# stella-cv/stella_vslam

Measured on NVIDIA H100. Metric: frames/sec (ORB+match+local BA) @1920x1080, 2000 kpts, higher is better.
Workload: dtype u8

## Files before the change

### stella_vslam_b200/csrc/lba_kernels.cu

```cuda
#include <algorithm>
#include <cmath>
#include <cstdlib>
#include <new>
#include <sched.h>

#include <chrono>
#include <memory>
#include <mutex>
#include <thread>
#include <vector>

#include "common.cuh"
#include "lm_common.cuh"
#include "quat.cuh"
#include "staging.cuh"
#include "track_chain.cuh"

namespace b200 {
namespace lba {

constexpr double kPi = 3.14159265358979323846;

struct Cam {
    int model;
// ... 773 lines not shown
                int x = 0, rem = tid;
                while (rem >= 6 - x) {
                    rem -= 6 - x;
                    ++x;
                }
                const int y = x + rem;
                W.Hpp[(size_t)i * 36 + x * 6 + y] = r;
                W.Hpp[(size_t)i * 36 + y * 6 + x] = r;
            } else {
                W.bp[(size_t)i * 6 + (tid - 21)] = r;
            }
        }
    }
    if (!last_cta_arrives(W.tickets, n_rows, &last_flag)) return;
    lm_after_build(W, stage);
}

__device__ __forceinline__ void dmma_m8n8k4(double& c0, double& c1, double a, double b) {
    asm volatile("mma.sync.aligned.m8n8k4.row.col.f64.f64.f64.f64 {%0,%1}, {%2}, {%3}, {%0,%1};" : "+d"(c0), "+d"(c1) : "d"(a), "d"(b));
}

__device__ __forceinline__ void schur_finish_block(const WinDev& W, const SchurBlock sb, double lambda, int lane) {
    const double* __restrict__ partials = W.chunk_part;
    double* __restrict__ M = W.M;
    const int n = W.n, ld = W.ld;
    for (int el = lane; el < 42; el += 32) {
        if (el >= 36 && sb.i != sb.j) continue;
        double sacc = 0.0;
        for (int c = sb.chunk_start; c < sb.chunk_end; ++c) sacc += __ldcg(partials + (size_t)c * 42 + el);
        if (el < 36) {
            const int r = el / 6, c = el - r * 6;
            double val = -sacc;
            if (sb.i == sb.j) val += W.Hpp[(size_t)sb.i * 36 + el] + (r == c ? lambda : 0.0);
            M[(size_t)(6 * sb.j + c) * ld + 6 * sb.i + r] = val;
            if (sb.i == sb.j) M[(size_t)(6 * sb.i + r) * ld + 6 * sb.j + c] = val;
        } else {
            const int r = el - 36;
            M[(size_t)n * ld + 6 * sb.i + r] = W.bp[(size_t)sb.i * 6 + r] - sacc;
        }
    }
}

__device__ void se3_oplus(const double* q, const double* t, const double* upd, double* qo, double* to) {
    const double* om = upd;
    const double* up = upd + 3;
    const double theta = sqrt(om[0] * om[0] + om[1] * om[1] + om[2] * om[2]);
    const double O[9] = {0, -om[2], om[1], om[2], 0, -om[0], -om[1], om[0], 0};
    double O2[9];
    for (int i = 0; i < 3; ++i)
        for (int j = 0; j < 3; ++j) O2[i * 3 + j] = O[i * 3] * O[j] + O[i * 3 + 1] * O[3 + j] + O[i * 3 + 2] * O[6 + j];
    double a, b, c, d;
    if (theta < 0.00001) {
        a = 1.0; b = 0.5; c = 0.5; d = 1.0 / 6.0;
    } else {
        a = sin(theta) / theta;
        b = (1 - cos(theta)) / (theta * theta);
        c = b;
        d = (theta - sin(theta)) / (theta * theta * theta);
    }
    double R[9], V[9];
    for (int i = 0; i < 9; ++i) {
        const double I = (i % 4 == 0) ? 1.0 : 0.0;
        R[i] = I + a * O[i] + b * O2[i];
        V[i] = I + c * O[i] + d * O2[i];
    }
    double dq[4], dt[3];
    rot_to_quat(R, dq);
    quat_normalize(dq);
    for (int i = 0; i < 3; ++i) dt[i] = V[i * 3] * up[0] + V[i * 3 + 1] * up[1] + V[i * 3 + 2] * up[2];
    double uv[3] = {dq[1] * t[2] - dq[2] * t[1], dq[2] * t[0] - dq[0] * t[2], dq[0] * t[1] - dq[1] * t[0]};
    uv[0] += uv[0]; uv[1] += uv[1]; uv[2] += uv[2];
    to[0] = dt[0] + t[0] + dq[3] * uv[0] + (dq[1] * uv[2] - dq[2] * uv[1]);
    to[1] = dt[1] + t[1] + dq[3] * uv[1] + (dq[2] * uv[0] - dq[0] * uv[2]);
    to[2] = dt[2] + t[2] + dq[3] * uv[2] + (dq[0] * uv[1] - dq[1] * uv[0]);
    double nq[4];
    nq[3] = dq[3] * q[3] - dq[0] * q[0] - dq[1] * q[1] - dq[2] * q[2];
    nq[0] = dq[3] * q[0] + dq[0] * q[3] + dq[1] * q[2] - dq[2] * q[1];
    nq[1] = dq[3] * q[1] + dq[1] * q[3] + dq[2] * q[0] - dq[0] * q[2];
    nq[2] = dq[3] * q[2] + dq[2] * q[3] + dq[0] * q[1] - dq[1] * q[0];
    quat_normalize(nq);
    qo[0] = nq[0]; qo[1] = nq[1]; qo[2] = nq[2]; qo[3] = nq[3];
}

constexpr int kCholThreads = 512;
constexpr int kNB = 24;
constexpr int kCholCluster = 8;

__device__ __forceinline__ unsigned cluster_ctarank() {
    unsigned r;
    asm volatile("mov.u32 %0, %%cluster_ctarank;" : "=r"(r));
    return r;
}
__device__ __forceinline__ unsigned cluster_nctarank() {
    unsigned r;
    asm volatile("mov.u32 %0, %%cluster_nctarank;" : "=r"(r));
    return r;
}
__device__ __forceinline__ void cluster_sync_all() {
    asm volatile("barrier.cluster.arrive.release.aligned;\n\tbarrier.cluster.wait.acquire.aligned;" ::: "memory");
}

__global__ void __launch_bounds__(kCholThreads) chol_solve_kernel(const WinDev* __restrict__ wins) {
    const unsigned crank = cluster_ctarank(), csize = cluster_nctarank();
    const WinDev& W = wins[blockIdx.x / csize];
    const LmCtl* __restrict__ ctl = W.ctl;
    if (!ctl->outer_go) return;
    const int n = W.n, ld = W.ld, K = W.K;
    double* __restrict__ M = W.M;
    const double* __restrict__ bp = W.bp;
    double* __restrict__ xp = W.xp;
    const int* __restrict__ pose_col = W.pose_col;
    double* __restrict__ result = W.r_result;
    int* __restrict__ fail = W.fail;
    extern __shared__ __align__(32) double dyn[];
    const double lambda = ctl->lambda;
    const int cur_idx = ctl->cur & 1;
    const double* __restrict__ q_cur = W.q[cur_idx];
    const double* __restrict__ t_cur = W.t[cur_idx];
    double* __restrict__ q_new = W.q[cur_idx ^ 1];
    double* __restrict__ t_new = W.t[cur_idx ^ 1];
    double* __restrict__ Rt_new = W.Rt[cur_idx ^ 1];
    double* D = dyn;
    double* Pn = dyn + kNB * (kNB + 1);
    const int mp = (n + 1 + 3) & ~3;
    __shared__ double xs[1024];
    __shared__ double invd_all[1024];
    __shared__ double sh[kCholThreads];
    __shared__ int bad;
    const int tid = threadIdx.x, nt = blockDim.x;
    const bool lead = crank == 0;
    if (tid == 0) bad = *fail;
    __syncthreads();
    long long t_diag = 0, t_panel = 0, t_trail = 0, t_back = 0, t0 = clock64(), t1;
#define PHASE(acc) do { t1 = clock64(); acc += t1 - t0; t0 = t1; } while (0)
    for (int kb = 0; kb < n && !bad; kb += kNB) {
        const int nb = min(kNB, n - kb);
        if (tid < 32) {
            double r[kNB];
#pragma unroll
            for (int k = 0; k < kNB; ++k) r[k] = (tid < nb && k <= tid) ? M[(size_t)(kb + tid) * ld + kb + k] : ((k == tid) ? 1.0 : 0.0);
            int b = 0;
#pragma unroll
            for (int j = 0; j < kNB; ++j) {
                const double djj = __shfl_sync(0xFFFFFFFFu, r[j], j);
                b |= (!(djj > 0.0) || !isfinite(djj)) ? 1 : 0;
                const double inv = rsqrt(djj), dd = djj * inv;
                if (tid == 0) invd_all[kb + j] = inv;
                r[j] = (tid == j) ? dd : ((tid > j) ? r[j] * inv : r[j]);
                const double mine = (tid > j) ? r[j] : 0.0;
#pragma unroll
                for (int k = j + 1; k < kNB; ++k) {
                    const double lkj = __shfl_sync(0xFFFFFFFFu, r[j], k);
                    r[k] = fma(-((tid >= k) ? mine : 0.0), lkj, r[k]);
                }
            }
            if (tid < kNB) {
#pragma unroll
                for (int k = 0; k < kNB; ++k) {
                    D[tid * (kNB + 1) + k] = r[k];
                }
            }
            if (tid == 0 && b) bad = 1;
        }
        __syncthreads();
        PHASE(t_diag);
        if (bad) break;
        const int r0 = kb + nb, m = n + 1 - r0;
        for (int t = tid; t < m; t += nt) {
            double* row = M + (size_t)(r0 + t) * ld + kb;
            double x[kNB];
#pragma unroll
            for (int j = 0; j < kNB; ++j) x[j] = (j < nb) ? row[j] : 0.0;
#pragma unroll
            for (int j = 0; j < kNB; ++j) {
                x[j] *= invd_all[kb + j];
#pragma unroll
                for (int k = j + 1; k < kNB; ++k) x[k] = fma(-x[j], D[k * (kNB + 1) + j], x[k]);
            }
#pragma unroll
            for (int j = 0; j < kNB; ++j) {
                Pn[(size_t)j * mp + t] = x[j];
            }
        }
        for (int idx = tid; idx < kNB * 4; idx += nt) {
            const int j = idx >> 2, t = m + (idx & 3);
            if (t < mp) Pn[(size_t)j * mp + t] = 0.0;
        }
        __syncthreads();
        PHASE(t_panel);
        const int tm = (m + 3) >> 2;
        const int n_tiles = tm * (tm + 1) / 2;
        for (int tile = tid * csize + crank; tile < n_tiles; tile += nt * csize) {
            int tr = (int)((sqrt(8.0 * tile + 1.0) - 1.0) * 0.5);
            while ((tr + 1) * (tr + 2) / 2 <= tile) ++tr;
            while (tr * (tr + 1) / 2 > tile) --tr;
            const int tc = tile - tr * (tr + 1) / 2;
            double acc[16];
#pragma unroll
            for (int a = 0; a < 16; ++a) acc[a] = 0.0;
            const int rb = tr * 4, cb = tc * 4;
#pragma unroll 4
            for (int k = 0; k < kNB; ++k) {
                const double2* pa = reinterpret_cast<const double2*>(Pn + (size_t)k * mp + rb);
                const double2* pb = reinterpret_cast<const double2*>(Pn + (size_t)k * mp + cb);
                const double2 a0 = pa[0], a1 = pa[1], b0 = pb[0], b1 = pb[1];
                const double a[4] = {a0.x, a0.y, a1.x, a1.y}, b[4] = {b0.x, b0.y, b1.x, b1.y};
#pragma unroll
                for (int u = 0; u < 4; ++u)
#pragma unroll
                    for (int w = 0; w < 4; ++w) acc[u * 4 + w] = fma(a[u], b[w], acc[u * 4 + w]);
            }
#pragma unroll
            for (int u = 0; u < 4; ++u)
#pragma unroll
                for (int w = 0; w < 4; ++w) {
                    const int r = rb + u, c = cb + w;
                    if (r < m && c <= r && r0 + c < n) M[(size_t)(r0 + r) * ld + r0 + c] -= acc[u * 4 + w];
                }
        }
        __syncthreads();
        if (csize > 1) cluster_sync_all();
        if (lead) {
            for (int idx = tid; idx < nb * nb; idx += nt) {
                const int i = idx / nb, j = idx - i * nb;
                if (j <= i) M[(size_t)(kb + i) * ld + kb + j] = D[i * (kNB + 1) + j];
            }
            for (int idx = tid; idx < m * nb; idx += nt) {
                const int t = idx / nb, j = idx - t * nb;
                M[(size_t)(r0 + t) * ld + kb + j] = Pn[(size_t)j * mp + t];
            }
        }
        __syncthreads();
        PHASE(t_trail);
    }
    if (!lead) return;
    if (bad) {
        if (tid == 0) {
            *fail = 1;
            result[0] = 0.0;
        }
    } else {
        for (int i = tid; i < n; i += nt) xs[i] = M[(size_t)n * ld + i];
        __syncthreads();
        for (int kb = ((n - 1) / kNB) * kNB; kb >= 0; kb -= kNB) {
            const int nb = min(kNB, n - kb);
            for (int idx = tid; idx < kNB * kNB; idx += nt) {
                const int i = idx / kNB, j = idx - i * kNB;
                D[i * (kNB + 1) + j] = (i < nb && j <= i) ? M[(size_t)(kb + i) * ld + kb + j] : 0.0;
            }
            __syncthreads();
            if (tid < 32) {
                double y = (tid < nb) ? xs[kb + tid] : 0.0;
#pragma unroll
                for (int j = kNB - 1; j >= 0; --j) {
                    const double xj = __shfl_sync(0xFFFFFFFFu, y, j) * ((j < nb) ? invd_all[kb + j] : 0.0);
                    if (tid == j) y = xj;
                    else if (tid < j) y = fma(-D[j * (kNB + 1) + tid], xj, y);
                }
                if (tid < nb) xs[kb + tid] = y;
            }
            __syncthreads();
            for (int i = tid; i < kb; i += nt) {
                double sacc = xs[i];
                for (int k = 0; k < nb; ++k) sacc = fma(-M[(size_t)(kb + k) * ld + i], xs[kb + k], sacc);
                xs[i] = sacc;
            }
            __syncthreads();
        }
        double sc = 0.0;
        for (int i = tid; i < n; i += nt) {
            xp[i] = xs[i];
            sc += xs[i] * (lambda * xs[i] + bp[i]);
        }
        const double tot = block_sum(sc, sh);
        PHASE(t_back);
        if (tid == 0) {
            result[0] = 1.0;
            result[1] = tot;
            result[2] = (double)t_diag;
            result[3] = (double)t_panel;
            result[4] = (double)t_trail;
            result[5] = (double)t_back;
        }
    }
#undef PHASE
    __syncthreads();
    for (int k = tid; k < K; k += nt) {
        double qn[4], tn[3];
        const int pc = pose_col[k];
        if (pc >= 0 && !bad) {
            se3_oplus(q_cur + 4 * k, t_cur + 3 * k, xs + 6 * pc, qn, tn);
        } else {
            for (int i = 0; i < 4; ++i) qn[i] = q_cur[4 * k + i];
            for (int i = 0; i < 3; ++i) tn[i] = t_cur[3 * k + i];
        }
        for (int i = 0; i < 4; ++i) q_new[4 * k + i] = qn[i];
        for (int i = 0; i < 3; ++i) t_new[3 * k + i] = tn[i];
        double R[9];
        quat_to_rot(qn, R);
        for (int i = 0; i < 9; ++i) Rt_new[12 * k + i] = R[i];
        for (int i = 0; i < 3; ++i) Rt_new[12 * k + 9 + i] = tn[i];
    }
}

constexpr int kSmmaKS = 100;
constexpr int kSmmaWarpDoubles = (6 + 7) * kSmmaKS;
__global__ void __launch_bounds__(128) schur_mma_kernel(const WinDev* __restrict__ wins) {
    extern __shared__ __align__(16) double smma[];
    const WinDev& W = wins[blockIdx.y];
    const LmCtl* ctl = W.ctl;
    if (!ctl->outer_go) return;
    const int warp = threadIdx.x >> 5, lane = threadIdx.x & 31;
    const int wid = blockIdx.x * 4 + warp;
    const int n_blocks = W.n_blocks, n_chunks = W.blk_chunk_start[n_blocks];
    if (wid >= n_chunks) {
        const int e = wid - n_chunks;
        if (e < n_blocks) {
            const SchurBlock sb = W.blocks[e];
            if (sb.chunk_start == sb.chunk_end) schur_finish_block(W, sb, ctl->lambda, lane);
        }
        return;
    }
    double* As = smma + (size_t)warp * kSmmaWarpDoubles;
    double* Bs = As + 6 * kSmmaKS;
    const SchurChunk ch = W.chunks[wid];
    const int Lf = W.Lf;
    const double* __restrict__ Hpl = W.Hpl;
    const double* __restrict__ Dinv = W.Dinv;
    const int g = lane >> 2, t4 = lane & 3;
    const double* a_row = As + min(g, 5) * kSmmaKS + t4;
    const double* b_row = Bs + min(g, 6) * kSmmaKS + t4;
    double c0 = 0.0, c1 = 0.0;
    for (int base = ch.start; base < ch.end; base += 32) {
        const int k = base + lane;
        const int np = min(32, ch.end - base);
        {
            double t[18], hc[18], b3[3];
            if (k < ch.end) {
                const int4 pr = W.pairs[k];
                double ra[12], rc[12], ha[18];
                load_hpl_record(Hpl + (size_t)pr.x * kHplStride, ra);
                load_hpl_record(Hpl + (size_t)pr.y * kHplStride, rc);
                expand_hpl(ra, ha);
                expand_hpl(rc, hc);
                const int lc = pr.z;
                const double D0 = Dinv[lc], D1 = Dinv[(size_t)Lf + lc], D2 = Dinv[(size_t)2 * Lf + lc];
                const double D4 = Dinv[(size_t)3 * Lf + lc], D5 = Dinv[(size_t)4 * Lf + lc], D8 = Dinv[(size_t)5 * Lf + lc];
#pragma unroll
                for (int r = 0; r < 6; ++r) {
                    t[r * 3] = ha[r * 3] * D0 + ha[r * 3 + 1] * D1 + ha[r * 3 + 2] * D2;
                    t[r * 3 + 1] = ha[r * 3] * D1 + ha[r * 3 + 1] * D4 + ha[r * 3 + 2] * D5;
                    t[r * 3 + 2] = ha[r * 3] * D2 + ha[r * 3 + 1] * D5 + ha[r * 3 + 2] * D8;
                }
                b3[0] = b3[1] = b3[2] = 0.0;
                if (ch.diag) {
                    b3[0] = W.bl[lc];
                    b3[1] = W.bl[(size_t)Lf + lc];
                    b3[2] = W.bl[(size_t)2 * Lf + lc];
                }
            } else {
#pragma unroll
                for (int i = 0; i < 18; ++i) t[i] = hc[i] = 0.0;
                b3[0] = b3[1] = b3[2] = 0.0;
            }
            double* ap = As + 3 * lane;
            double* bp2 = Bs + 3 * lane;
#pragma unroll
            for (int r = 0; r < 6; ++r)
#pragma unroll
                for (int kk = 0; kk < 3; ++kk) {
                    ap[r * kSmmaKS + kk] = t[r * 3 + kk];
                    bp2[r * kSmmaKS + kk] = hc[r * 3 + kk];
                }
#pragma unroll
            for (int kk = 0; kk < 3; ++kk) bp2[6 * kSmmaKS + kk] = b3[kk];
        }
        __syncwarp();
        const int steps = (3 * np + 3) >> 2;
#pragma unroll 4
        for (int s2 = 0; s2 < steps; ++s2) dmma_m8n8k4(c0, c1, a_row[4 * s2], b_row[4 * s2]);
        __syncwarp();
    }
    double* part = W.chunk_part + (size_t)wid * 42;
    if (g < 6) {
        if (t4 < 3) {
// ... 838 lines not shown
        }
        if (K) std::memcpy(hs + o.pose_col, h.pose_col.data(), sizeof(int) * K);
        if (L) {
            std::memcpy(hs + o.pt_col, h.pt_col.data(), sizeof(int) * L);
            std::memcpy(hs + o.pts0, P.points, sizeof(double) * 3 * L);
        }
        double* q0 = reinterpret_cast<double*>(hs + o.q0);
        double* t0 = reinterpret_cast<double*>(hs + o.t0);
        double* Rt0 = reinterpret_cast<double*>(hs + o.Rt0);
        for (size_t k = 0; k < K; ++k) {
            const double* M = P.pose_cw + 16 * k;
            const double R[9] = {M[0], M[1], M[2], M[4], M[5], M[6], M[8], M[9], M[10]};
            rot_to_quat(R, &q0[4 * k]);
            quat_normalize(&q0[4 * k]);
            t0[3 * k] = M[3]; t0[3 * k + 1] = M[7]; t0[3 * k + 2] = M[11];
            quat_to_rot(&q0[4 * k], &Rt0[12 * k]);
            Rt0[12 * k + 9] = M[3]; Rt0[12 * k + 10] = M[7]; Rt0[12 * k + 11] = M[11];
        }
        WinDev& W = hwd[x];
        std::memset(&W, 0, sizeof(W));
        W.K = h.K; W.L = h.L; W.E = h.E; W.Kf = h.Kf; W.Lf = h.Lf; W.n = h.n; W.ld = h.ld; W.n_cams = P.n_cams; W.lbc = h.lbc;
        W.e_pose = (const int*)(d + o.e_pose); W.e_point = (const int*)(d + o.e_point); W.e_cam = d + o.e_cam; W.e_robust = d + o.e_robust;
        W.e_can_outlier = d + o.e_can; W.e_obs = (const float*)(d + o.e_obs); W.e_isig = (const float*)(d + o.e_isig);
        W.e_delta = (const float*)(d + o.e_delta); W.pose_col = (const int*)(d + o.pose_col); W.pt_col = (const int*)(d + o.pt_col);
        W.cams = (const Cam*)(d + o.cams);
        W.pt_cnt = (int*)(d + o.pt_cnt); W.pt_start = (int*)(d + o.pt_start); W.order = (int*)(d + o.order); W.edges = (EdgeS*)(d + o.edges);
        W.epcol = (int*)(d + o.epcol); W.pose_cnt = (int*)(d + o.pose_cnt); W.pose_start = (int*)(d + o.pose_start);
        W.pose_edges = (int*)(d + o.pose_edges); W.level = d + o.level; W.robust = d + o.robust;
        W.rowrec = (int4*)(d + o.rowrec);
        W.lm_mask = (unsigned long long*)(d + o.lm_mask); W.mask_words = h.mask_words; W.n_blocks = h.n_blocks; W.blk_cnt = (int*)(d + o.blk_cnt);
        W.blk_pair_start = (int*)(d + o.blk_pair_start); W.blk_chunk_start = (int*)(d + o.blk_chunk_start); W.pairs = (int4*)(d + o.pairs);
        W.blocks = (SchurBlock*)(d + o.blocks); W.chunks = (SchurChunk*)(d + o.chunks); W.chunk_part = (double*)(d + o.chunk_part);
        W.blk_done = (int*)(d + o.blk_done);
        W.q[0] = (double*)(d + o.q0); W.q[1] = (double*)(d + o.q1); W.t[0] = (double*)(d + o.t0); W.t[1] = (double*)(d + o.t1);
        W.Rt[0] = (double*)(d + o.Rt0); W.Rt[1] = (double*)(d + o.Rt1); W.pts[0] = (double*)(d + o.pts0); W.pts[1] = (double*)(d + o.pts1);
        W.chi[0] = (double*)(d + o.chi0); W.chi[1] = (double*)(d + o.chi1);
        W.Hpl = (double*)(d + o.Hpl); W.Hll = (double*)(d + o.Hll); W.bl = (double*)(d + o.bl); W.Dinv = (double*)(d + o.Dinv);
        W.Hpp = (double*)(d + o.Hpp); W.bp = (double*)(d + o.bp); W.M = (double*)(d + o.M); W.xp = (double*)(d + o.xp);
        W.gP = (double*)(d + o.gP); W.gD = (double*)(d + o.gD); W.ginvd = (double*)(d + o.ginvd);
        W.r_chi = (double*)(d + o.r_chi); W.r_diag = (double*)(d + o.r_diag); W.r_scale = (double*)(d + o.r_scale); W.r_result = (double*)(d + o.r_result);
        W.fail = (int*)(d + o.fail); W.tickets = (int*)(d + o.tickets); W.bad_input = (int*)(d + o.bad);
        W.ctl = (LmCtl*)(d + o_ctl) + x;
        W.qf = (double*)(d + o.qf); W.tf = (double*)(d + o.tf); W.pf = (double*)(d + o.pf); W.out = d + o.out;
        LmCtl& c = hctl0[x];
        std::memset(&c, 0, sizeof(c));
        c.ok = 1;
        S.h_abort[x] = 0;
        c.abort_word = (stops && stops[act[x]]) ? S.d_abort + x : nullptr;
    }
    if (debug) fprintf(stderr, "[lba] %d windows staged in %.3f ms (upload %.2f MB, arena %.1f MB)\n", nw, ms_since(t_begin), upload_bytes / 1e6, cv.end / 1e6);
    cudaStream_t st = S.stream;
    int launches = 0;
    S.prof_kind.clear();
    auto mark = [&](int kind) -> int {
        if (!S.profile) return B200_OK;
        const size_t idx = S.prof_kind.size();
        if (idx >= S.prof_ev.size()) {
            cudaEvent_t e;
            B200_CUDA(cudaEventCreate(&e));
            S.prof_ev.push_back(e);
        }
        B200_CUDA(cudaEventRecord(S.prof_ev[idx], st));
        S.prof_kind.push_back(kind);
        return B200_OK;
    };
    B200_CUDA(cudaEventRecord(S.ev0, st));
    B200_CUDA(S.arena.upload(upload_bytes, st));
    B200_CUDA(cudaMemsetAsync(d + upload_bytes, 0, zero_end - upload_bytes, st));
    if ((rc = mark(-1))) return rc;
    const WinDev* wins = (const WinDev*)(d + o_wins);
    const LmCtl* d_ctl = (const LmCtl*)(d + o_ctl);
    plan_count_kernel<<<dim3(ceil_div(maxE, 256), nw), 256, 0, st>>>(wins);
    plan_scan_kernel<<<nw, 1024, 0, st>>>(wins);
    plan_place_kernel<<<dim3(ceil_div(maxE, 256), nw), 256, 0, st>>>(wins);
    plan_sort_kernel<<<dim3(ceil_div(maxL, 128), nw), 128, 0, st>>>(wins);
    plan_pose_lists_kernel<<<dim3(maxKf, nw), kListThreads, 0, st>>>(wins);
    plan_pairs_kernel<false><<<dim3(ceil_div(max_blocks, 4), nw), 128, 0, st>>>(wins);
    plan_pair_scan_kernel<<<nw, 1024, 0, st>>>(wins);
    plan_pairs_kernel<true><<<dim3(ceil_div(max_blocks, 4), nw), 128, 0, st>>>(wins);
    launches += 8;
    if ((rc = mark(0))) return rc;
    B200_RANGE("b200:lba:rounds+export");
    const bool large = max_n > kCholOnChipMax || S.force_offchip;
    const size_t chol_smem = sizeof(double) * ((size_t)kNB * (kNB + 1) + 4 + (size_t)((std::min(max_n, kCholOnChipMax) + 1 + 3) & ~3) * kNB);
    B200_CUDA(cudaFuncSetAttribute(chol_solve_kernel, cudaFuncAttributeMaxDynamicSharedMemorySize, (int)chol_smem));
    const int chol_cluster = S.chol_cluster_pinned ? S.chol_cluster : (nw <= 2 ? 8 : 4);
    auto launch_rep = [&]() -> int {
        int rcm;
        landmark_kernel<kBuild><<<dim3(max_lbc, nw), kLmThreads, 0, st>>>(wins);
        if ((rcm = mark(1))) return rcm;
        pose_rows_kernel<<<dim3(maxKf, nw), kRowThreads, 0, st>>>(wins);
        if ((rcm = mark(2))) return rcm;
        schur_mma_kernel<<<dim3(ceil_div(max_chunk_warps, 4), nw), 128, 4 * kSmmaWarpDoubles * sizeof(double), st>>>(wins);
        if ((rcm = mark(3))) return rcm;
        if (large) {
            for (int kb = 0; kb < max_n; kb += kNB) {
                const int m = max_n + 1 - std::min(kb + kNB, max_n);
                const long long tm = (m + 3) >> 2, n_tiles = tm * (tm + 1) / 2;
                gchol_panel_kernel<<<dim3(ceil_div(m + 4, kGcholThreads), nw), kGcholThreads, 0, st>>>(wins, kb);
                gchol_trail_kernel<<<dim3((unsigned)std::max<long long>(1, (n_tiles + kGcholThreads - 1) / kGcholThreads), nw), kGcholThreads, 0, st>>>(wins, kb);
                launches += 2;
            }
            gchol_finish_kernel<<<nw, kGfinThreads, 0, st>>>(wins);
        } else {
            cudaLaunchConfig_t cfg = {};
            cfg.gridDim = dim3(chol_cluster * nw);
            cfg.blockDim = dim3(kCholThreads);
            cfg.dynamicSmemBytes = chol_smem;
            cfg.stream = st;
            cudaLaunchAttribute attr[1];
            attr[0].id = cudaLaunchAttributeClusterDimension;
            attr[0].val.clusterDim.x = chol_cluster;
            attr[0].val.clusterDim.y = 1;
            attr[0].val.clusterDim.z = 1;
            cfg.attrs = attr;
            cfg.numAttrs = 1;
            B200_CUDA(cudaLaunchKernelEx(&cfg, chol_solve_kernel, wins));
        }
        if ((rcm = mark(4))) return rcm;
        backsub_kernel<<<dim3(max_lbc, nw), 128, 0, st>>>(wins);
        if ((rcm = mark(5))) return rcm;
        launches += 5;
        return B200_OK;
    };
    auto fetch_issue = [&](int b) -> int {
        B200_CUDA(cudaMemcpyAsync(h_ctl2[b], d_ctl, sizeof(LmCtl) * nw, cudaMemcpyDeviceToHost, st));
        B200_CUDA(cudaEventRecord(S.ev_ctl[b], st));
        return B200_OK;
    };
    auto fetch_wait = [&](int b) -> int {
        B200_CUDA(S.wait_event(S.ev_ctl[b]));
        h_ctl = h_ctl2[b];
        for (int x = 0; x < nw; ++x)
            if (stops && stops[act[x]] && *stops[act[x]]) S.h_abort[x] = 1;
        return B200_OK;
    };
    auto fetch_ctl = [&]() -> int {
        int r_ = fetch_issue(0);
        return r_ ? r_ : fetch_wait(0);
    };
    const int iters[2] = {iters1, iters2};
    int rc2;
    for (int r = 0; r < rounds; ++r) {
        if (r == 1) {
            if ((rc2 = fetch_ctl())) return rc2;
            for (int x = 0; x < nw; ++x) {
                volatile uint8_t* f = stops ? stops[act[x]] : nullptr;
                if (!f) continue;
                if (h_ctl[x].stop_flag || *f) {
                    S.h_abort[x] = 1;
                    *f = 1;
                } else {
                    S.h_abort[x] = 0;
                }
            }
        }
        lm_round_begin_kernel<<<ceil_div(nw, 64), 64, 0, st>>>(wins, nw, iters[r], r, gain_thr);
        ++launches;
        if (r == 1) {
            outlier_kernel<<<dim3(ceil_div(maxE, 128), nw), 128, 0, st>>>(wins, 0);
            ++launches;
        }
        if (iters[r] > 0) {
            int need = iters[r];
            for (;;) {
                const int chunk = std::max(1, std::min(need, 6));
                for (int i = 0; i < chunk; ++i)
                    if ((rc2 = launch_rep())) return rc2;
                if ((rc2 = fetch_ctl())) return rc2;
                need = 0;
                for (int x = 0; x < nw; ++x)
                    if (h_ctl[x].outer_go) need = std::max(need, std::max(1, h_ctl[x].iterations - h_ctl[x].it));
                if (need == 0) break;
            }
        }
        landmark_kernel<kRoundEnd><<<dim3(max_lbc, nw), kLmThreads, 0, st>>>(wins);
        lm_round_end_kernel<<<nw, 256, 0, st>>>(wins, r);
        launches += 2;
    }
    if (rounds == 2) outlier_kernel<<<dim3(ceil_div(maxE, 128), nw), 128, 0, st>>>(wins, 1);
    lm_export_kernel<<<dim3(ceil_div(std::max(std::max(4 * maxK, 3 * maxL), 1), 256), nw), 256, 0, st>>>(wins);
    launches += 2;
    B200_CUDA(cudaGetLastError());
    if ((rc = mark(7))) return rc;
    B200_CUDA(cudaEventRecord(S.ev1, st));
    B200_CUDA(cudaMemcpyAsync(h_export, d + export_begin, export_bytes, cudaMemcpyDeviceToHost, st));
    std::vector<int> h_bad(nw, 0);
    if ((rc2 = fetch_ctl())) return rc2;
    for (int x = 0; x < nw; ++x) B200_CUDA(cudaMemcpyAsync(&h_bad[x], d + wo[x].bad, sizeof(int), cudaMemcpyDeviceToHost, st));
    B200_CUDA(cudaStreamSynchronize(st));
    B200_CUDA(cudaEventElapsedTime(&S.last_ms, S.ev0, S.ev1));
    S.last_launches = launches;
    for (int k2 = 0; k2 < 8; ++k2) {
        S.prof_ms[k2] = 0.f;
        S.prof_n[k2] = 0;
    }
    for (size_t m = 1; m < S.prof_kind.size(); ++m) {
        float ms = 0.f;
        B200_CUDA(cudaEventElapsedTime(&ms, S.prof_ev[m - 1], S.prof_ev[m]));
        const int kd = S.prof_kind[m];
        if (kd >= 0 && kd < 8) {
            S.prof_ms[kd] += ms;
            S.prof_n[kd] += 1;
        }
    }
    if (debug) fprintf(stderr, "[lba] batch of %d windows: %.3f ms wall, %.3f ms on the stream, %d launches\n", nw, ms_since(t_begin), S.last_ms, launches);
    for (int x = 0; x < nw; ++x) {
        const int w = act[x];
        const HostWin& h = hw[x];
        const b200_lba_problem_t& P = Ps[w];
        const WinOff& o = wo[x];
        if (h_bad[x]) {
            set_error("b200_lba_solve: edge %d of window %d references an invalid vertex/camera", h_bad[x] - 1, w);
            status[w] = B200_ERR_INVALID;
            ret = B200_ERR_INVALID;
            continue;
        }
        const LmCtl& c = h_ctl[x];
        if (stats) {
            stats[w].lambda_init = c.lambda_init;
            for (int r = 0; r < 2; ++r) {
                stats[w].iterations[r] = c.iters_done[r];
                stats[w].chi2[r] = c.chi2[r];
                stats[w].lambda_final[r] = c.lambda_final[r];
            }
        }
        if (stops && stops[w] && c.stop_flag) *stops[w] = 1;
        S.last_gain_stop = c.stop_flag != 0;
        const unsigned char* ex = h_export + (o.qf - export_begin);
        const double* qf = reinterpret_cast<const double*>(ex);
        const double* tf = reinterpret_cast<const double*>(h_export + (o.tf - export_begin));
        const double* pf = reinterpret_cast<const double*>(h_export + (o.pf - export_begin));
        const unsigned char* out = h_export + (o.out - export_begin);
        int n_out = 0;
        for (int e = 0; e < h.E && rounds == 2; ++e) n_out += out[e];
        if (rounds == 2 && outlier_outs && outlier_outs[w] && h.E) std::memcpy(outlier_outs[w], out, h.E);
        if (stats) stats[w].n_outliers = n_out;
        if (h.L) std::memcpy(points_outs[w], pf, sizeof(double) * 3 * (size_t)h.L);
        for (int k = 0; k < h.K; ++k) {
            double* M = pose_outs[w] + 16 * (size_t)k;
            if (P.pose_fixed[k]) {
                std::memcpy(M, P.pose_cw + 16 * (size_t)k, sizeof(double) * 16);
                continue;
            }
            double R[9];
            quat_to_rot(&qf[4 * k], R);
            M[0] = R[0]; M[1] = R[1]; M[2] = R[2]; M[3] = tf[3 * k];
            M[4] = R[3]; M[5] = R[4]; M[6] = R[5]; M[7] = tf[3 * k + 1];
            M[8] = R[6]; M[9] = R[7]; M[10] = R[8]; M[11] = tf[3 * k + 2];
            M[12] = 0; M[13] = 0; M[14] = 0; M[15] = 1;
        }
    }
    return ret;
}

constexpr int kTrackEdgeThreads = 256;
constexpr int kMatchedBias = 1 << 30;
__global__ void __launch_bounds__(kTrackEdgeThreads) track_edges_kernel(chain::TrackShared sh, const chain::TrackFrameDev* __restrict__ frames,
                                                                        PoseProb* __restrict__ probs, PoseEdge* __restrict__ edges_all,
                                                                        int* __restrict__ edge_kp_all) {
    __shared__ int warp_sum[kTrackEdgeThreads / 32];
    __shared__ int s_base;
    const chain::TrackFrameDev& F = frames[blockIdx.x];
    const int tid = threadIdx.x, lane = tid & 31, warp = tid >> 5;
    const int n = F.status[0];
    int* slot = F.kp_landmark_out;
    for (int i = tid; i < F.kp_cap; i += kTrackEdgeThreads) {
        int l = -1;
        if (i < n && F.kp_landmark && i < F.n_kp_in) {
            l = F.kp_landmark[i];
            if (l < 0 || l >= F.n_lm) l = -1;
        }
        slot[i] = l;
        F.kp_outlier[i] = 0;
    }
    __syncthreads();
    for (int q = tid; q < F.n_lm; q += kTrackEdgeThreads) {
        const int k = F.match_out[q];
        if (k >= 0 && k < n) atomicMax(&slot[k], q + kMatchedBias);
    }
    __syncthreads();
    if (tid == 0) s_base = 0;
    const PoseProb pb = probs[blockIdx.x];
    PoseEdge* __restrict__ edges = edges_all + pb.edge_off;
    int* __restrict__ edge_kp = edge_kp_all + pb.edge_off;
    __syncthreads();
    for (int i0 = 0; i0 < n; i0 += kTrackEdgeThreads) {
        const int i = i0 + tid;
        int l = -1;
// ... 345 lines not shown
```

Baseline: 10130.

## Add shared-memory-resident two-CTA cluster Cholesky for small reduced systems

Adds a Cholesky kernel for reduced camera systems up to a size threshold. The lower triangle is held as 8x8 tiles in distributed shared memory, split by tile row across a two-CTA cluster. Panel rows are mirrored into the peer CTA's buffer, and the trailing update uses DMMA m8n8k4 tensor-core ops with split arrive/wait so local work overlaps the cluster barrier. This is meant to remove repeated global-memory traffic on the Schur matrix during factorization, at the cost of more shared memory, cluster barriers and more complex indexing. Pose-update code is factored into a helper, and a debug printout of cycle counts is added.

```diff
diff --git a/stella_vslam_b200/csrc/lba_kernels.cu b/stella_vslam_b200/csrc/lba_kernels.cu
--- a/stella_vslam_b200/csrc/lba_kernels.cu
+++ b/stella_vslam_b200/csrc/lba_kernels.cu
@@ -879,6 +879,31 @@
     qo[0] = nq[0]; qo[1] = nq[1]; qo[2] = nq[2]; qo[3] = nq[3];
 }
 
+__device__ void trial_states(const WinDev& W, const double* xs, bool solved) {
+    const int cur_idx = W.ctl->cur & 1;
+    const double* __restrict__ q_cur = W.q[cur_idx];
+    const double* __restrict__ t_cur = W.t[cur_idx];
+    double* __restrict__ q_new = W.q[cur_idx ^ 1];
+    double* __restrict__ t_new = W.t[cur_idx ^ 1];
+    double* __restrict__ Rt_new = W.Rt[cur_idx ^ 1];
+    for (int k = threadIdx.x; k < W.K; k += blockDim.x) {
+        double qn[4], tn[3];
+        const int pc = W.pose_col[k];
+        if (pc >= 0 && solved) {
+            se3_oplus(q_cur + 4 * k, t_cur + 3 * k, xs + 6 * pc, qn, tn);
+        } else {
+            for (int i = 0; i < 4; ++i) qn[i] = q_cur[4 * k + i];
+            for (int i = 0; i < 3; ++i) tn[i] = t_cur[3 * k + i];
+        }
+        for (int i = 0; i < 4; ++i) q_new[4 * k + i] = qn[i];
+        for (int i = 0; i < 3; ++i) t_new[3 * k + i] = tn[i];
+        double R[9];
+        quat_to_rot(qn, R);
+        for (int i = 0; i < 9; ++i) Rt_new[12 * k + i] = R[i];
+        for (int i = 0; i < 3; ++i) Rt_new[12 * k + 9 + i] = tn[i];
+    }
+}
+
 constexpr int kCholThreads = 512;
 constexpr int kNB = 24;
 constexpr int kCholCluster = 8;
@@ -895,6 +920,38 @@
 }
 __device__ __forceinline__ void cluster_sync_all() {
     asm volatile("barrier.cluster.arrive.release.aligned;\n\tbarrier.cluster.wait.acquire.aligned;" ::: "memory");
+}
+__device__ __forceinline__ void cluster_arrive() { asm volatile("barrier.cluster.arrive.release.aligned;" ::: "memory"); }
+__device__ __forceinline__ void cluster_wait() { asm volatile("barrier.cluster.wait.acquire.aligned;" ::: "memory"); }
+__device__ __forceinline__ double* cluster_map(double* p, unsigned rank) {
+    unsigned long long q;
+    asm volatile("mapa.u64 %0, %1, %2;" : "=l"(q) : "l"(p), "r"(rank));
+    return reinterpret_cast<double*>(q);
+}
+
+__device__ __forceinline__ bool diag_block_factor(double (&r)[kNB], int lane, double* invd, double* D) {
+    int b = 0;
+#pragma unroll
+    for (int j = 0; j < kNB; ++j) {
+        const double djj = __shfl_sync(0xFFFFFFFFu, r[j], j);
+        b |= (!(djj > 0.0) || !isfinite(djj)) ? 1 : 0;
+        const double inv = rsqrt(djj), dd = djj * inv;
+        if (lane == 0) invd[j] = inv;
+        r[j] = (lane == j) ? dd : ((lane > j) ? r[j] * inv : r[j]);
+        const double mine = (lane > j) ? r[j] : 0.0;
+#pragma unroll
+        for (int k = j + 1; k < kNB; ++k) {
+            const double lkj = __shfl_sync(0xFFFFFFFFu, r[j], k);
+            r[k] = fma(-((lane >= k) ? mine : 0.0), lkj, r[k]);
+        }
+    }
+    if (lane < kNB) {
+#pragma unroll
+        for (int k = 0; k < kNB; ++k) {
+            D[lane * (kNB + 1) + k] = r[k];
+        }
+    }
+    return b != 0;
 }
 
 __global__ void __launch_bounds__(kCholThreads) chol_solve_kernel(const WinDev* __restrict__ wins) {
@@ -902,21 +959,14 @@
     const WinDev& W = wins[blockIdx.x / csize];
     const LmCtl* __restrict__ ctl = W.ctl;
     if (!ctl->outer_go) return;
-    const int n = W.n, ld = W.ld, K = W.K;
+    const int n = W.n, ld = W.ld;
     double* __restrict__ M = W.M;
     const double* __restrict__ bp = W.bp;
     double* __restrict__ xp = W.xp;
-    const int* __restrict__ pose_col = W.pose_col;
     double* __restrict__ result = W.r_result;
     int* __restrict__ fail = W.fail;
     extern __shared__ __align__(32) double dyn[];
     const double lambda = ctl->lambda;
-    const int cur_idx = ctl->cur & 1;
-    const double* __restrict__ q_cur = W.q[cur_idx];
-    const double* __restrict__ t_cur = W.t[cur_idx];
-    double* __restrict__ q_new = W.q[cur_idx ^ 1];
-    double* __restrict__ t_new = W.t[cur_idx ^ 1];
-    double* __restrict__ Rt_new = W.Rt[cur_idx ^ 1];
     double* D = dyn;
     double* Pn = dyn + kNB * (kNB + 1);
     const int mp = (n + 1 + 3) & ~3;
@@ -936,28 +986,7 @@
             double r[kNB];
 #pragma unroll
             for (int k = 0; k < kNB; ++k) r[k] = (tid < nb && k <= tid) ? M[(size_t)(kb + tid) * ld + kb + k] : ((k == tid) ? 1.0 : 0.0);
-            int b = 0;
-#pragma unroll
-            for (int j = 0; j < kNB; ++j) {
-                const double djj = __shfl_sync(0xFFFFFFFFu, r[j], j);
-                b |= (!(djj > 0.0) || !isfinite(djj)) ? 1 : 0;
-                const double inv = rsqrt(djj), dd = djj * inv;
-                if (tid == 0) invd_all[kb + j] = inv;
-                r[j] = (tid == j) ? dd : ((tid > j) ? r[j] * inv : r[j]);
-                const double mine = (tid > j) ? r[j] : 0.0;
-#pragma unroll
-                for (int k = j + 1; k < kNB; ++k) {
-                    const double lkj = __shfl_sync(0xFFFFFFFFu, r[j], k);
-                    r[k] = fma(-((tid >= k) ? mine : 0.0), lkj, r[k]);
-                }
-            }
-            if (tid < kNB) {
-#pragma unroll
-                for (int k = 0; k < kNB; ++k) {
-                    D[tid * (kNB + 1) + k] = r[k];
-                }
-            }
-            if (tid == 0 && b) bad = 1;
+            if (diag_block_factor(r, tid, invd_all + kb, D) && tid == 0) bad = 1;
         }
         __syncthreads();
         PHASE(t_diag);
@@ -1082,22 +1111,224 @@
     }
 #undef PHASE
     __syncthreads();
-    for (int k = tid; k < K; k += nt) {
-        double qn[4], tn[3];
-        const int pc = pose_col[k];
-        if (pc >= 0 && !bad) {
-            se3_oplus(q_cur + 4 * k, t_cur + 3 * k, xs + 6 * pc, qn, tn);
-        } else {
-            for (int i = 0; i < 4; ++i) qn[i] = q_cur[4 * k + i];
-            for (int i = 0; i < 3; ++i) tn[i] = t_cur[3 * k + i];
-        }
-        for (int i = 0; i < 4; ++i) q_new[4 * k + i] = qn[i];
-        for (int i = 0; i < 3; ++i) t_new[3 * k + i] = tn[i];
-        double R[9];
-        quat_to_rot(qn, R);
-        for (int i = 0; i < 9; ++i) Rt_new[12 * k + i] = R[i];
-        for (int i = 0; i < 3; ++i) Rt_new[12 * k + 9 + i] = tn[i];
-    }
+    trial_states(W, xs, !bad);
+}
+
+constexpr int kResCluster = 2;
+constexpr int kCholResidentMax = 288;
+constexpr int kResRows = kCholResidentMax + kNB;
+
+__host__ __device__ __forceinline__ int res_tile_off(int i, int rank) {
+    const int k = (i - rank) >> 1;
+    return k * k + k * rank;
+}
+__host__ __device__ __forceinline__ int res_tix(int r, int c) { return r * 8 + (c ^ ((r & 2) << 1)); }
+__device__ __forceinline__ int tri_row(int t, int b) {
+    int a = (int)((sqrtf((float)(b * b + 4 * t)) - (float)b) * 0.5f);
+    while ((a + 1) * (a + 1) + (a + 1) * b <= t) ++a;
+    while (a > 0 && a * a + a * b > t) --a;
+    return a;
+}
+
+static size_t chol_resident_smem(int n) {
+    const int T0 = (n + 7) / 8;
+    int own = 0;
+    for (int rank = 0; rank < kResCluster; ++rank) {
+        int c = 0;
+        for (int i = rank; i <= T0; i += kResCluster) c += i < T0 ? i + 1 : T0;
+        own = std::max(own, c);
+    }
+    return sizeof(double) * 64 * ((size_t)3 * (T0 / 2 + 1) + own);
+}
+
+__global__ void __launch_bounds__(kCholThreads) chol_resident_kernel(const WinDev* __restrict__ wins) {
+    const int crank = (int)cluster_ctarank();
+    const WinDev& W = wins[blockIdx.x / kResCluster];
+    const LmCtl* __restrict__ ctl = W.ctl;
+    if (!ctl->outer_go) return;
+    const int n = W.n, ld = W.ld;
+    const double* __restrict__ M = W.M;
+    const double* __restrict__ bp = W.bp;
+    double* __restrict__ xp = W.xp;
+    double* __restrict__ result = W.r_result;
+    int* __restrict__ fail = W.fail;
+    const double lambda = ctl->lambda;
+    extern __shared__ __align__(32) double dyn[];
+    __shared__ double D[kNB * (kNB + 1)];
+    __shared__ double invd_all[kResRows];
+    __shared__ double xs[kResRows];
+    __shared__ double sh[kCholThreads];
+    __shared__ int bad;
+    const int T0 = (n + 7) >> 3;
+    double* xbuf = dyn;
+    double* tiles = dyn + (size_t)3 * 64 * (T0 / 2 + 1);
+    double* peer_xbuf = cluster_map(xbuf, crank ^ 1);
+    double* peer_tiles = cluster_map(tiles, crank ^ 1);
+    auto tile_of = [&](int i, int c) -> double* {
+        return ((i & 1) == crank ? tiles : peer_tiles) + (size_t)(res_tile_off(i, i & 1) + c) * 64;
+    };
+    const int tid = threadIdx.x, nt = blockDim.x, warp = tid >> 5, lane = tid & 31, nwarps = nt >> 5;
+    const int g = lane >> 2, t4 = lane & 3;
+    const bool lead = crank == 0;
+    if (tid == 0) bad = *fail;
+    long long t_diag = 0, t_panel = 0, t_trail = 0, t_back = 0, t0 = clock64(), t1;
+#define PHASE(acc) do { t1 = clock64(); acc += t1 - t0; t0 = t1; } while (0)
+    const int last_row = T0 - ((T0 - crank) & 1);
+    const int n_own = last_row < crank ? 0 : res_tile_off(last_row, crank) + (last_row < T0 ? last_row + 1 : T0);
+    for (int tb = warp; tb < n_own; tb += 4 * nwarps) {
+        double v[8];
+#pragma unroll
+        for (int u = 0; u < 4; ++u) {
+            const int t = tb + u * nwarps;
+            const int k = tri_row(t, crank), i = crank + 2 * k, c = t - res_tile_off(i, crank);
+#pragma unroll
+            for (int h = 0; h < 2; ++h) {
+                const int r = (lane >> 3) + 4 * h, R = 8 * i + r, C = 8 * c + (lane & 7);
+                double x = 0.0;
+                if (t < n_own) {
+                    if (i == T0) x = (r == 0 && C < n) ? M[(size_t)n * ld + C] : 0.0;
+                    else x = (R < n && C <= R) ? M[(size_t)R * ld + C] : (R == C ? 1.0 : 0.0);
+                }
+                v[2 * u + h] = x;
+            }
+        }
+#pragma unroll
+        for (int u = 0; u < 4; ++u) {
+            const int t = tb + u * nwarps;
+            if (t < n_own)
+#pragma unroll
+                for (int h = 0; h < 2; ++h) tiles[(size_t)t * 64 + res_tix((lane >> 3) + 4 * h, lane & 7)] = v[2 * u + h];
+        }
+    }
+    cluster_sync_all();
+    PHASE(t_panel);
+    for (int c0 = 0; c0 < T0 && !bad; c0 += 3) {
+        const int nbt = min(3, T0 - c0), kb = 8 * c0, nb = 8 * nbt, i1 = c0 + nbt;
+        if (tid < 32) {
+            double r[kNB];
+            const double* row = tid < nb ? tile_of(c0 + (tid >> 3), c0) : nullptr;
+#pragma unroll
+            for (int k = 0; k < kNB; ++k) r[k] = (tid < nb && k <= tid) ? row[(k >> 3) * 64 + res_tix(tid & 7, k & 7)] : ((k == tid) ? 1.0 : 0.0);
+            if (diag_block_factor(r, tid, invd_all + kb, D) && tid == 0) bad = 1;
+        }
+        __syncthreads();
+        PHASE(t_diag);
+        if (bad) break;
+        const int i0 = i1 + ((i1 ^ crank) & 1);
+        const int n_rows = i0 <= T0 ? (T0 - i0) / 2 + 1 : 0;
+        for (int t = tid; t < 8 * n_rows; t += nt) {
+            const int i = i0 + 2 * (t >> 3), rr = t & 7;
+            double* tp = tiles + (size_t)(res_tile_off(i, crank) + c0) * 64;
+            double* pp = peer_xbuf + (size_t)(i >> 1) * 3 * 64;
+            double x[kNB];
+#pragma unroll
+            for (int j = 0; j < kNB; ++j) x[j] = (j < nb) ? tp[(j >> 3) * 64 + res_tix(rr, j & 7)] : 0.0;
+#pragma unroll
+            for (int j = 0; j < kNB; ++j) {
+                x[j] *= invd_all[kb + j];
+#pragma unroll
+                for (int k = j + 1; k < kNB; ++k) x[k] = fma(-x[j], D[k * (kNB + 1) + j], x[k]);
+            }
+#pragma unroll
+            for (int j = 0; j < kNB; ++j) {
+                if (j < nb) {
+                    const int e = (j >> 3) * 64 + res_tix(rr, j & 7);
+                    tp[e] = x[j];
+                    pp[e] = x[j];
+                }
+            }
+        }
+        __syncthreads();
+        cluster_arrive();
+        PHASE(t_panel);
+        const int lb = i0 - i1;
+        const int n_trail = n_rows == 0 ? 0 : (n_rows - 1) * (n_rows - 1) + (n_rows - 1) * lb + (min(i0 + 2 * (n_rows - 1), T0 - 1) - i1 + 1);
+        for (int pass = 0; pass < 2; ++pass) {
+            if (pass == 1) cluster_wait();
+            for (int t = warp; t < n_trail; t += nwarps) {
+                const int a = tri_row(t, lb), i = i0 + 2 * a, j = i1 + t - (a * a + a * lb);
+                const bool own_j = ((j ^ crank) & 1) == 0;
+                if (own_j != (pass == 0)) continue;
+                const double* at = tiles + (size_t)(res_tile_off(i, crank) + c0) * 64;
+                const double* bt = own_j ? tiles + (size_t)(res_tile_off(j, crank) + c0) * 64 : xbuf + (size_t)(j >> 1) * 3 * 64;
+                double s0 = 0.0, s1 = 0.0;
+#pragma unroll
+                for (int s = 0; s < 6; ++s) {
+                    if (s < 2 * nbt) {
+                        const int e = (s >> 1) * 64 + res_tix(g, 4 * (s & 1) + t4);
+                        dmma_m8n8k4(s0, s1, at[e], bt[e]);
+                    }
+                }
+                double2* cp = reinterpret_cast<double2*>(tiles + (size_t)(res_tile_off(i, crank) + j) * 64 + res_tix(g, 2 * t4));
+                double2 cv = *cp;
+                cv.x -= s0;
+                cv.y -= s1;
+                *cp = cv;
+            }
+        }
+        for (int idx = tid; idx < nb * nb; idx += nt) {
+            const int i = idx / nb, j = idx - i * nb, ti = c0 + (i >> 3);
+            if (j <= i && (ti & 1) == crank) tiles[(size_t)(res_tile_off(ti, crank) + c0 + (j >> 3)) * 64 + res_tix(i & 7, j & 7)] = D[i * (kNB + 1) + j];
+        }
+        cluster_sync_all();
+        PHASE(t_trail);
+    }
+    if (lead && !bad) {
+        for (int i = tid; i < n; i += nt) xs[i] = tile_of(T0, i >> 3)[res_tix(0, i & 7)];
+        __syncthreads();
+        for (int kb = ((n - 1) / kNB) * kNB; kb >= 0; kb -= kNB) {
+            const int nb = min(kNB, n - kb), c0 = kb >> 3;
+            for (int idx = tid; idx < kNB * kNB; idx += nt) {
+                const int i = idx / kNB, j = idx - i * kNB;
+                D[i * (kNB + 1) + j] = (i < nb && j <= i) ? tile_of(c0 + (i >> 3), c0 + (j >> 3))[res_tix(i & 7, j & 7)] : 0.0;
+            }
+            __syncthreads();
+            if (tid < 32) {
+                double y = (tid < nb) ? xs[kb + tid] : 0.0;
+#pragma unroll
+                for (int j = kNB - 1; j >= 0; --j) {
+                    const double xj = __shfl_sync(0xFFFFFFFFu, y, j) * ((j < nb) ? invd_all[kb + j] : 0.0);
+                    if (tid == j) y = xj;
+                    else if (tid < j) y = fma(-D[j * (kNB + 1) + tid], xj, y);
+                }
+                if (tid < nb) xs[kb + tid] = y;
+            }
+            __syncthreads();
+            for (int i = tid; i < kb; i += nt) {
+                double sacc = xs[i];
+                for (int k = 0; k < nb; ++k) sacc = fma(-tile_of(c0 + (k >> 3), i >> 3)[res_tix(k & 7, i & 7)], xs[kb + k], sacc);
+                xs[i] = sacc;
+            }
+            __syncthreads();
+        }
+    }
+    cluster_sync_all();
+    if (!lead) return;
+    if (bad) {
+        if (tid == 0) {
+            *fail = 1;
+            result[0] = 0.0;
+        }
+    } else {
+        double sc = 0.0;
+        for (int i = tid; i < n; i += nt) {
+            xp[i] = xs[i];
+            sc += xs[i] * (lambda * xs[i] + bp[i]);
+        }
+        const double tot = block_sum(sc, sh);
+        PHASE(t_back);
+        if (tid == 0) {
+            result[0] = 1.0;
+            result[1] = tot;
+            result[2] = (double)t_diag;
+            result[3] = (double)t_panel;
+            result[4] = (double)t_trail;
+            result[5] = (double)t_back;
+        }
+    }
+#undef PHASE
+    __syncthreads();
+    trial_states(W, xs, !bad);
 }
 
 constexpr int kSmmaKS = 100;
@@ -2102,8 +2333,11 @@
     if ((rc = mark(0))) return rc;
     B200_RANGE("b200:lba:rounds+export");
     const bool large = max_n > kCholOnChipMax || S.force_offchip;
+    const bool resident = !large && max_n <= kCholResidentMax;
     const size_t chol_smem = sizeof(double) * ((size_t)kNB * (kNB + 1) + 4 + (size_t)((std::min(max_n, kCholOnChipMax) + 1 + 3) & ~3) * kNB);
+    const size_t res_smem = chol_resident_smem(std::min(max_n, kCholResidentMax));
     B200_CUDA(cudaFuncSetAttribute(chol_solve_kernel, cudaFuncAttributeMaxDynamicSharedMemorySize, (int)chol_smem));
+    B200_CUDA(cudaFuncSetAttribute(chol_resident_kernel, cudaFuncAttributeMaxDynamicSharedMemorySize, (int)res_smem));
     const int chol_cluster = S.chol_cluster_pinned ? S.chol_cluster : (nw <= 2 ? 8 : 4);
     auto launch_rep = [&]() -> int {
         int rcm;
@@ -2123,19 +2357,21 @@
             }
             gchol_finish_kernel<<<nw, kGfinThreads, 0, st>>>(wins);
         } else {
+            const int csize = resident ? kResCluster : chol_cluster;
             cudaLaunchConfig_t cfg = {};
-            cfg.gridDim = dim3(chol_cluster * nw);
+            cfg.gridDim = dim3(csize * nw);
             cfg.blockDim = dim3(kCholThreads);
-            cfg.dynamicSmemBytes = chol_smem;
+            cfg.dynamicSmemBytes = resident ? res_smem : chol_smem;
             cfg.stream = st;
             cudaLaunchAttribute attr[1];
             attr[0].id = cudaLaunchAttributeClusterDimension;
-            attr[0].val.clusterDim.x = chol_cluster;
+            attr[0].val.clusterDim.x = csize;
             attr[0].val.clusterDim.y = 1;
             attr[0].val.clusterDim.z = 1;
             cfg.attrs = attr;
             cfg.numAttrs = 1;
-            B200_CUDA(cudaLaunchKernelEx(&cfg, chol_solve_kernel, wins));
+            if (resident) B200_CUDA(cudaLaunchKernelEx(&cfg, chol_resident_kernel, wins));
+            else B200_CUDA(cudaLaunchKernelEx(&cfg, chol_solve_kernel, wins));
         }
         if ((rcm = mark(4))) return rcm;
         backsub_kernel<<<dim3(max_lbc, nw), 128, 0, st>>>(wins);
@@ -2225,6 +2461,11 @@
         }
     }
     if (debug) fprintf(stderr, "[lba] batch of %d windows: %.3f ms wall, %.3f ms on the stream, %d launches\n", nw, ms_since(t_begin), S.last_ms, launches);
+    for (int x = 0; debug && !large && x < nw; ++x) {
+        double rr[8];
+        B200_CUDA(cudaMemcpy(rr, d + wo[x].r_result, sizeof(rr), cudaMemcpyDeviceToHost));
+        fprintf(stderr, "[lba] window %d cholesky cycles: diag %.0f panel %.0f trail %.0f back %.0f\n", x, rr[2], rr[3], rr[4], rr[5]);
+    }
     for (int x = 0; x < nw; ++x) {
         const int w = act[x];
         const HostWin& h = hw[x];
```

New measurement: 10340, median of 6. 1.02x the previous value.
